# hccho2/Tacotron-Wavenet-Vocoder-Korean

Measured on AMD Instinct MI355X. Metric: WaveNet autoregressive audio samples/sec at 24 kHz, batch=8, higher is better.
Workload: dtype f32

## Files before the change

### tacotron-wavenet-vocoder-korean_amd/csrc/twv_wavenet_xcd.hip

```cpp
#include <hip/hip_runtime.h>
#include <stdint.h>
#include <string>
#include <type_traits>
#include "../../include/twv_amd.h"
#include "twv_layout.hpp"
#include "twv_math.hpp"
#include "twv_dev.hpp"
#include "twv_dpp.hpp"
#include "twv_categorical.hpp"
#include "twv_xcd.hpp"

using namespace twv;

#ifndef TWV_CHAIN_PAD
#define TWV_CHAIN_PAD 0
#endif
#ifndef TWV_WATCHDOG_LOG2
#define TWV_WATCHDOG_LOG2 21
#endif
#define TWV_STR2(x) #x
#define TWV_STR(x) TWV_STR2(x)
namespace {

typedef __attribute__((address_space(1))) unsigned long long gu64;
// ... 23 lines not shown
    return xb_load(rs, uword, lword);
}
__device__ __forceinline__ unsigned long long xbm_load(rsrc_t rs, int uword, int lword) { return xb_load_t<true>(rs, uword, lword); }
__device__ __forceinline__ u32x4s xbm_load2(rsrc_t rs, int uword, int lpair)
{
    asm volatile("" ::: "memory");
    return xb_load2(rs, uword, lpair);
}
__device__ __forceinline__ void xb_store(rsrc_t rs, int uword, int lword, unsigned tag, float v)
{
    __builtin_amdgcn_raw_buffer_store_b64(u32x2v{__float_as_uint(v), tag}, rs, lword * 8, uword * 8, kAuxStore);
    asm volatile("" ::: "memory");
}
__device__ __forceinline__ void xb_store2(rsrc_t rs, int uword, int lane, unsigned tag, float va, float vb)
{
    const u32x4s d = {__float_as_uint(va), tag, __float_as_uint(vb), tag};
    __builtin_amdgcn_raw_buffer_store_b128(d, rs, lane * 16, uword * 8, kAuxStore);
    asm volatile("s_nop 1" ::"v"(d) : "memory");
}
__device__ __forceinline__ unsigned g_tag(unsigned long long q) { return (unsigned)(q >> 32); }
__device__ __forceinline__ float g_val(unsigned long long q) { return __uint_as_float((unsigned)q); }

struct Poll {
    rsrc_t rs;
    int* status;
    int it;
    bool dead;
};
template <bool BAR = false>
__device__ __forceinline__ bool poll_tick(Poll& p, int code)
{
    if (p.dead) return false;
    if (((++p.it) & 63) == 0) {
        if (xb_load_t<BAR>(p.rs, (int)XcdExch::CTRL + 1, 0) != 0ull) { p.dead = true; return false; }
        if (p.it > (1 << TWV_WATCHDOG_LOG2)) {
            atomicMax(p.status, code);
            xb_store(p.rs, (int)XcdExch::CTRL + 1, 0, 1u, 0.0f);
            p.dead = true;
            return false;
        }
    }
    return true;
}
__device__ __forceinline__ void nap_until(unsigned long long target)
{
#pragma nounroll
    for (int i = 0; i < 4096 && __builtin_amdgcn_s_memtime() < target; ++i) __builtin_amdgcn_s_sleep(8);
}

__device__ __forceinline__ int lane_of_z(int k) { return ((k & 2) ? 16 : 0) + 2 * (k >> 2) + (k & 1); }
__device__ __forceinline__ int lane_of_x(int j) { return j < 16 ? j : 16 + j; }

struct ChainRegs { float wc[32]; float bd; };

#define XSTAMP(cond_, slot_) do { if ((INSTR & 1) && a.prof != nullptr && b == a.prof_stream && t < a.prof_steps && lane == 0 && (cond_)) a.prof[(long long)t * 64 + (slot_)] = wall_clock64(); } while (0)

#define WACC_DECL() unsigned long long wacc_[6] = {0, 0, 0, 0, 0, 0}, w0_ = 0, wt0_ = 0; if (INSTR & 4) wt0_ = __builtin_amdgcn_s_memtime()
#define WACC_T0() do { if (INSTR & 4) w0_ = __builtin_amdgcn_s_memtime(); } while (0)
#define WACC_T1(i_) do { if (INSTR & 4) wacc_[i_] += __builtin_amdgcn_s_memtime() - w0_; } while (0)
constexpr int kTraceStep = 2000;
#define WTRACE(cond_, slot_) do { if ((INSTR & 4) && a.prof != nullptr && t == kTraceStep && (cond_) && lane == 0) a.prof[2048 + (slot_)] = wall_clock64(); } while (0)
#define WACC_OUT(prof_, slot_, wave_) do { if ((INSTR & 4) && (prof_) != nullptr && (slot_) >= 0 && lane == 0) {                 \
        unsigned long long* o_ = (prof_) + (((slot_) * 8 + (wave_)) * 8);                                                        \
        o_[0] = __builtin_amdgcn_s_memtime() - wt0_;                                                                             \
        o_[1] = wacc_[0]; o_[2] = wacc_[1]; o_[3] = wacc_[2]; o_[4] = wacc_[3]; o_[5] = wacc_[4]; o_[6] = wacc_[5]; } } while (0)
#define XMARK(role_, stage_) do { if ((INSTR & 1) && lane == 0) xb_store(rs, (int)XcdExch::MARK + (role_) * 8 + (int)(threadIdx.x >> 6), 0, (unsigned)t + 1u, (float)(stage_)); } while (0)

enum { ROLE_CHAIN = 0, ROLE_SERVICE = 1, ROLE_SKIP0 = 2, ROLE_CONV0 = 10, ROLE_LC0 = 18 };
constexpr int kXcdStreamsPerXcd = kXcdStreams / 8;

struct XArgs {
    XcdLaunch p;
    int n_lc_wg, lc_lpw;
    int total_roles;
};

template <int NS> struct XStreams { rsrc_t rs[NS]; int b[NS]; };
__device__ __forceinline__ rsrc_t exch_rsrc(const XcdLaunch& a, int b)
{
    return __builtin_amdgcn_make_buffer_rsrc(a.exch + (long long)b * XcdExch::WORDS, 0, (int)(XcdExch::WORDS * 8), 0x00020000);
}
struct XLazyRs { const XcdLaunch* a; int xcc, ns; __device__ __forceinline__ rsrc_t operator[](int k) const { return exch_rsrc(*a, xcc + 8 * (k < ns ? k : 0)); } };
struct XLazyB { int xcc, ns; __device__ __forceinline__ int operator[](int k) const { return xcc + 8 * (k < ns ? k : 0); } };
template <int NS> struct XStreamsLazy { XLazyRs rs; XLazyB b; };
constexpr int kSkipLdsWords = 32 * 64;
constexpr int kConvLdsFloats = 16 * 64 + 64;

template <int INSTR, bool ALL, bool FORCED, bool SEG1, bool TWOSEG, int NC, bool ONEHOT = false, int HW = -1>
__device__ __forceinline__ void chain_role(const XArgs& xa, int b, rsrc_t rs)
{
    const XcdLaunch& a = xa.p;
    const Layout& L = a.lay;
    const int w = __builtin_amdgcn_readfirstlane(threadIdx.x >> 6), lane = threadIdx.x & 63;
    const int NL = L.NL, T = a.T;
    const bool use_bias = L.use_bias != 0, has_gc = L.G > 0, has_lc = L.L > 0;
    constexpr bool forced = FORCED;
    const int l0 = SEG1 ? kXcdSeg0Layers + 4 * w : (w < 6 ? 4 * w : 24 + 3 * (w - 6));
    const int lw0 = SEG1 ? 4 * w : l0;
    const int cap = SEG1 ? 4 : (w < 6 ? 4 : 3);
    int nl = NL - l0;
    nl = nl < 0 ? 0 : (nl > cap ? cap : nl);
    const int nlc = NC >= 0 ? NC : nl;
    const bool next_has = (l0 + nl < NL);
    const bool head = HW >= 0 ? (HW == 1) : (!SEG1 && (w == 7));
    const bool to_seg1 = TWOSEG && !SEG1 && w == 7 && next_has;
    constexpr bool two_seg = TWOSEG;
    if (nl == 0 && !head) return;
    const int oc = dpp_conv_out(lane), od = dpp_dense_out(lane);
    const ActCoef coef = act_coef(lane >= 32);
    float* stb = a.state + (long long)b * L.state_stride;
    Poll pl{rs, a.status, 0, false};
    constexpr int O_WD = 2048;

    ChainRegs W[4];
#pragma unroll
    for (int i = 0; i < 4; ++i) {
        if (i < nl) {
            const f32x4* src = reinterpret_cast<const f32x4*>(a.P + L.off_xl + (long long)(l0 + i) * kXcdXlFloats) + lane;
#pragma unroll
            for (int q = 0; q < 8; ++q) { const f32x4 v = src[q * 64]; W[i].wc[4 * q] = v.x; W[i].wc[4 * q + 1] = v.y; W[i].wc[4 * q + 2] = v.z; W[i].wc[4 * q + 3] = v.w; }
#pragma unroll
            for (int q = 0; q < 4; ++q) LDS4((O_WD >> 2) + ((lw0 + i) * 4 + q) * 64 + lane) = src[(8 + q) * 64];
            const f32x4 v = src[12 * 64];
            W[i].bd = dense_bias_init(lane, use_bias ? v.y : 0.0f);
        }
    }
    float ha = 0.0f, hb = 0.0f, first_in = 0.0f, b2v = 0.0f, s_lnl = 0.0f, s_tq = 0.0f, samp = 0.0f;
    float cp[4] = {0.0f, 0.0f, 0.0f, 0.0f};
    int q_prev = 0, q_valid = 0, samp_q = 0, first_q = 0;
    float w0row = 0.0f;
    double u_next = 0.0;
    const int chx = dpp_dense_out(lane);
    const bool sampler = head && !forced;
    const bool is15 = (lane & 15) == 15;
    auto causal_prepare = [&]() {
        const float t1 = __int_as_float(__builtin_amdgcn_update_dpp(0, __float_as_int(ha), 0x101, 0xf, 0xf, true));
        const float b0 = __int_as_float(__builtin_amdgcn_update_dpp(0, __float_as_int(hb), 0x150, 0xf, 0xf, true));
        ha = is15 ? b0 : t1;
        hb = __int_as_float(__builtin_amdgcn_update_dpp(0, __float_as_int(hb), 0x101, 0xf, 0xf, true));
        causal_partial_dpp(W[3].wc, ha, hb, cp);
    };
    auto noise = [&](int t) {
        const float* up = a.uniforms + ((long long)b * T + t) * (L.nr_mix + 1);
        const float u = lane <= L.nr_mix ? up[lane] : 0.5f;
        s_lnl = log_e(-log_e(u));
        const float uu = __shfl(u, L.nr_mix);
        s_tq = log_e(uu) - log_e(1.0f - uu);
    };
    if (head) {
        if constexpr (ONEHOT) {
            const int* meta = reinterpret_cast<const int*>(stb + L.st_meta);
            q_valid = __builtin_amdgcn_readfirstlane(meta[M_PREV_VALID]);
            q_prev = __builtin_amdgcn_readfirstlane(meta[M_QPREV]) & (L.Q - 1);
            w0row = a.P[L.off_causal + (long long)q_prev * 32 + chx];
            if (!forced) first_q = reinterpret_cast<const int*>(a.first_input)[b];
        } else {
            const f32x4* src = reinterpret_cast<const f32x4*>(a.P + L.off_xc) + lane;
#pragma unroll
            for (int q = 0; q < 8; ++q) { const f32x4 v = src[q * 64]; W[3].wc[4 * q] = v.x; W[3].wc[4 * q + 1] = v.y; W[3].wc[4 * q + 2] = v.z; W[3].wc[4 * q + 3] = v.w; }
            ha = stb[L.st_hist + (lane & 15)];
            hb = stb[L.st_hist + 16 + (lane & 15)];
            if (!forced) first_in = reinterpret_cast<const float*>(a.first_input)[b];
            if (sampler && use_bias && lane < L.O) b2v = a.P[L.off_b2 + lane];
            causal_prepare();
        }
    }
    __builtin_amdgcn_s_waitcnt(0);
    asm volatile(".p2align 6\n\t.rept " TWV_STR(TWV_CHAIN_PAD) "\n\ts_nop 0\n\t.endr" ::: "memory");

    float X = 0.0f;
    unsigned long long t_in = 0, in_period = 0, now_in = 0;
    for (int t = 0; t < T && !pl.dead; ++t) {
        asm volatile(".p2align 6");
        const unsigned tag = (unsigned)t + 1u;
        if (head) {
            if (forced && t > 0) {
                pl.it = 0;
                for (;;) {
                    const unsigned long long q = two_seg ? xb_load(rs, (int)XcdExch::DONE, lane) : LDSU64(8 * 64 + lane);
                    if (__all(g_tag(q) == (unsigned)t)) break;
                    if (!poll_tick(pl, 35)) break;
                    __builtin_amdgcn_s_sleep(2);
                }
                if (pl.dead) break;
            }
            XSTAMP(true, 0);
            if constexpr (ONEHOT) {
                const int q_raw = forced ? reinterpret_cast<const int*>(a.forced)[(long long)b * T + t] : (t == 0 ? first_q : samp_q);
                const int q_in = __builtin_amdgcn_readfirstlane(q_raw) & (L.Q - 1);
                const float w1row = a.P[L.off_causal + ((long long)L.Q + q_in) * 32 + chx];
                const float x0 = q_valid ? w0row + w1row : w1row;
                LDSU64(0 * 64 + lane) = ((unsigned long long)tag << 32) | (unsigned long long)__float_as_uint(x0);
                XSTAMP(true, 1);
                if (lane == 0) {
                    if (sampler && t > 0) reinterpret_cast<int*>(a.out)[(long long)b * T + t - 1] = samp_q;
                    xb_store(rs, (int)XcdExch::CTRL, 0, tag, 0.0f);
                }
                q_prev = q_in; q_valid = 1;
                w0row = a.P[L.off_causal + (long long)q_in * 32 + chx];
                if (sampler) u_next = reinterpret_cast<const double*>(a.uniforms)[(long long)b * T + t];
            } else {
            const float s_in = forced ? reinterpret_cast<const float*>(a.forced)[(long long)b * T + t] : (t == 0 ? first_in : samp);
            const float c3 = fma_(W[3].wc[31], s_in, cp[3]);
            const float x0 = (cp[0] + cp[1]) + (cp[2] + c3);
            LDSU64(0 * 64 + lane) = ((unsigned long long)tag << 32) | (unsigned long long)__float_as_uint(x0);
            XSTAMP(true, 1);
            if (lane == 0) {
                if (sampler && t > 0) a.out[(long long)b * T + t - 1] = samp;
                xb_store(rs, (int)XcdExch::CTRL, 0, tag, 0.0f);
            }
            hb = is15 ? s_in : hb;
            if (t + 1 < T) causal_prepare();
            if (sampler) noise(t);
            }
            __builtin_amdgcn_s_setprio(0);
        }
        XMARK(SEG1 ? 30 : ROLE_CHAIN, 1);
        float pre[4] = {0.0f, 0.0f, 0.0f, 0.0f};
        if (nlc > 0) {
            pl.it = 0;
            for (;;) {
                bool ok = true;
#pragma unroll
                for (int i = 0; i < 4; ++i) {
                    if (i < nlc) {
                        const unsigned long long qp = xb_load(rs, (int)XcdExch::PG + (l0 + i) * 64, oc);
                        ok = ok && g_tag(qp) == tag;
                        pre[i] = g_val(qp);
                    }
                }
                if (__all(ok)) break;
                if (!poll_tick(pl, 31)) break;
                __builtin_amdgcn_s_sleep(4);
            }
            XSTAMP(!SEG1, 26 + w);
            XMARK(SEG1 ? 30 : ROLE_CHAIN, 2);
            if (in_period) nap_until(t_in + in_period - (in_period >> 4));
            unsigned long long q;
            pl.it = 0;
            if (SEG1 && w == 0) {
                for (;;) {
                    q = xb_load(rs, (int)XcdExch::SEG, lane);
                    if (__all(g_tag(q) == tag)) break;
                    if (!poll_tick(pl, 36)) break;
                }
            } else {
                for (;;) {
                    q = LDSU64(w * 64 + lane);
                    if (__all(g_tag(q) == tag)) break;
                    if (!poll_tick(pl, 33)) break;
                }
            }
            __builtin_amdgcn_s_setprio(3);
            X = g_val(q);
            now_in = __builtin_amdgcn_s_memtime();
            XSTAMP(true, (SEG1 ? 40 : 2) + w);
            XMARK(SEG1 ? 30 : ROLE_CHAIN, 3);
        }
        constexpr bool DEFER = ALL && !FORCED && !SEG1 && NC > 0 && HW == 0;
        float zs[4] = {0.0f, 0.0f, 0.0f, 0.0f}, xs[4] = {0.0f, 0.0f, 0.0f, 0.0f};
        auto run_layers = [&](auto nc) {
            constexpr int N = decltype(nc)::value;
#pragma unroll
            for (int i = 0; i < N; ++i) {
                float wd[16];
#pragma unroll
                for (int q = 0; q < 4; ++q) {
                    const f32x4 v = LDS4((O_WD >> 2) + ((lw0 + i) * 4 + q) * 64 + lane);
                    wd[4 * q] = v.x; wd[4 * q + 1] = v.y; wd[4 * q + 2] = v.z; wd[4 * q + 3] = v.w;
                }
                const float z = layer_front_dpp(W[i].wc, coef, X, pre[i]);
                if (DEFER) { zs[i] = z; xs[i] = X; }
                else xb_store2(rs, (int)XcdExch::ZX + (l0 + i) * 128, lane, tag, z, X);
                layer_back_dpp(wd, W[i].bd, z, X);
                if ((INSTR & 2) && a.dbg != nullptr && t < a.dbg_steps) {
                    float* dp = a.dbg + ((long long)b * a.dbg_steps + t) * ((long long)NL * 64 + L.Opad) + (long long)(l0 + i) * 64;
                    if (lane < 32) dp[dpp_z_index(lane)] = z;
                    if ((lane & 16) == 0) dp[32 + od] = X;
                }
            }
        };
        if constexpr (NC > 0) run_layers(std::integral_constant<int, NC>{});
        else {
            if (nl == 4) run_layers(std::integral_constant<int, 4>{});
            else if (nl == 3) run_layers(std::integral_constant<int, 3>{});
            else if (nl == 2) run_layers(std::integral_constant<int, 2>{});
            else if (nl == 1) run_layers(std::integral_constant<int, 1>{});
        }
        if (to_seg1) xb_store(rs, (int)XcdExch::SEG, lane, tag, X);
        else if (nlc > 0) LDSU64((next_has ? w + 1 : 9) * 64 + lane) = ((unsigned long long)tag << 32) | (unsigned long long)__float_as_uint(X);
        XSTAMP(DEFER && nl > 0, (SEG1 ? 48 : 10) + w);
        if (DEFER) {
#pragma unroll
            for (int i = 0; i < (NC > 0 ? NC : 0); ++i) xb_store2(rs, (int)XcdExch::ZX + (l0 + i) * 128, lane, tag, zs[i], xs[i]);
        }
        if (forced && nl > 0 && !next_has) {
            if (SEG1) xb_store(rs, (int)XcdExch::DONE, lane, tag, 0.0f);
            else LDSU64(8 * 64 + lane) = (unsigned long long)tag << 32;
        }
        if (nlc > 0) {
            const unsigned long long d = now_in - t_in;
            in_period = (t_in != 0 && d < (1ull << 18)) ? d : 0;
            t_in = now_in;
        }
        if (!sampler) __builtin_amdgcn_s_setprio(0);
        XSTAMP(!DEFER && nl > 0, (SEG1 ? 48 : 10) + w);
        XMARK(SEG1 ? 30 : ROLE_CHAIN, 4);
        if constexpr (ONEHOT) {
          if (sampler) {
            __builtin_amdgcn_s_setprio(3);
            u32x4s d0, d1;
            pl.it = 0;
            for (;;) {
                d0 = xb_load2(rs, (int)XcdExch::QL, lane * 2);
                d1 = xb_load2(rs, (int)XcdExch::QL, lane * 2 + 1);
                if (__all(d0.y == tag && d0.w == tag && d1.y == tag && d1.w == tag)) break;
                if (!poll_tick(pl, 34)) break;
            }
            XSTAMP(true, 18);
            XMARK(SEG1 ? 30 : ROLE_CHAIN, 5);
            const float y[4] = {__uint_as_float(d0.x), __uint_as_float(d0.z), __uint_as_float(d1.x), __uint_as_float(d1.z)};
            if ((INSTR & 2) && a.dbg != nullptr && t < a.dbg_steps) {
#pragma unroll
                for (int k = 0; k < 4; ++k)
                    a.dbg[((long long)b * a.dbg_steps + t) * ((long long)NL * 64 + L.Opad) + (long long)NL * 64 + lane + 64 * k] = y[k];
            }
            bool bad_p = false;
            samp_q = categorical_sample<4>(y, L.Q, lane, a.temperature, u_next, nullptr,
                                           ((INSTR & 1) && a.prof != nullptr && b == a.prof_stream && t < a.prof_steps) ? a.prof + (long long)t * 64 + 38 : nullptr, &bad_p);
            if (bad_p && lane == 0) atomicMax(a.status, 31);
            XSTAMP(true, 19);
          }
        } else
        if (sampler) {
            __builtin_amdgcn_s_setprio(3);
            const int half = lane >> 5;
            unsigned long long q[8];
            pl.it = 0;
            for (;;) {
                bool good = true;
#pragma unroll
                for (int k = 0; k < 4; ++k) {
                    const u32x4s d = xb_load2(rs, (int)XcdExch::PT, (half * 4 + k) * 32 + (lane & 31));
                    q[2 * k] = ((unsigned long long)d.y << 32) | d.x;
                    q[2 * k + 1] = ((unsigned long long)d.w << 32) | d.z;
                    good = good && d.y == tag && d.w == tag;
                }
                if (__all(good)) break;
                if (!poll_tick(pl, 34)) break;
            }
            XSTAMP(true, 18);
            XMARK(SEG1 ? 30 : ROLE_CHAIN, 5);
            float y = g_val(q[0]);
#pragma unroll
            for (int k = 1; k < 8; ++k) y = y + g_val(q[k]);
#pragma unroll
            for (int k = 0; k < 8; ++k) {
                const auto sw = __builtin_amdgcn_permlane32_swap((unsigned)q[k], (unsigned)q[k], false, false);
                y = y + __uint_as_float(sw[1]);
            }
            if (use_bias && lane < L.O) y = y + b2v;
            if ((INSTR & 2) && a.dbg != nullptr && t < a.dbg_steps)
                a.dbg[((long long)b * a.dbg_steps + t) * ((long long)NL * 64 + L.Opad) + (long long)NL * 64 + lane] = y;
            const int nr = L.nr_mix;
            const float lsmin = (float)-32.23619130191664;
            const float e_all = exp_e(y > lsmin ? y : lsmin);
            const float ninf = __uint_as_float(0xff800000u);
            const float gmb = (lane < nr) ? y - s_lnl : ninf;
            float mx = gmb;
            mx = fmaxf(mx, __int_as_float(__builtin_amdgcn_update_dpp(__float_as_int(ninf), __float_as_int(mx), 0x111, 0xf, 0xf, false)));
            mx = fmaxf(mx, __int_as_float(__builtin_amdgcn_update_dpp(__float_as_int(ninf), __float_as_int(mx), 0x112, 0xf, 0xf, false)));
            mx = fmaxf(mx, __int_as_float(__builtin_amdgcn_update_dpp(__float_as_int(ninf), __float_as_int(mx), 0x114, 0xf, 0xf, false)));
            mx = fmaxf(mx, __int_as_float(__builtin_amdgcn_update_dpp(__float_as_int(ninf), __float_as_int(mx), 0x118, 0xf, 0xf, false)));
            const float best = __int_as_float(__builtin_amdgcn_readlane(__float_as_int(mx), 15));
            const unsigned long long hit = __ballot(lane < nr && gmb == best);
            const int k = hit ? (int)__ffsll((long long)hit) - 1 : 0;
            const float mean = __int_as_float(__builtin_amdgcn_readlane(__float_as_int(y), nr + k));
            const float e = __int_as_float(__builtin_amdgcn_readlane(__float_as_int(e_all), 2 * nr + k));
            const float prod = e * s_tq;
            float xs = mean + prod;
            xs = xs > -1.0f ? xs : -1.0f;
            xs = xs < 1.0f ? xs : 1.0f;
            samp = xs;
            XSTAMP(true, 19);
        }
    }

    if (head) {
        if constexpr (ONEHOT) {
            if (lane == 0) {
                if (sampler && !pl.dead && T > 0) reinterpret_cast<int*>(a.out)[(long long)b * T + T - 1] = samp_q;
                int* meta = reinterpret_cast<int*>(stb + L.st_meta);
                meta[M_TABS] = meta[M_TABS] + T;
                meta[M_PREV_VALID] = q_valid;
                meta[M_QPREV] = q_prev;
            }
        } else {
        if (sampler && !pl.dead && T > 0 && lane == 0) a.out[(long long)b * T + T - 1] = samp;
        if (lane < 16) stb[L.st_hist + lane] = ha;
        else if (lane < 32) stb[L.st_hist + lane] = hb;
        if (lane == 0) {
            int* meta = reinterpret_cast<int*>(stb + L.st_meta);
            meta[M_TABS] = meta[M_TABS] + T;
// ... 692 lines not shown
            lds[o_cur + lane] = rowa[k];
            lds[o_cur + 64 + lane] = rowb[k];
            if (mode != XLC_UPSAMPLED) {
#pragma unroll
                for (int i = 0; i < 4; ++i) {
                    if (i < n_up) {
                        const int o_nxt = (o_cur == o_row) ? o_row + 128 : o_row;
#pragma unroll
                        for (int hlf = 0; hlf < 2; ++hlf) {
                            const int m = hlf * 64 + lane;
                            const float x0 = lds[o_cur + m];
                            const float x1 = m > 0 ? lds[o_cur + m - 1] : 0.0f;
                            const float s0 = fma_(k0[i], x0, 0.0f);
                            const float s1 = fma_(k1[i], x1, 0.0f);
                            const float r = (s0 + s1) + (0.0f + 0.0f);
                            lds[o_nxt + m] = m < Lc ? r : 0.0f;
                        }
                        o_cur = o_nxt;
                    }
                }
            }
            float resx[kLt];
#pragma unroll
            for (int idx = 0; idx < kLt; ++idx) {
                resx[idx] = 0.0f;
                if (idx < nown * NLC) {
                    const int j = idx / NLC, c = idx - j * NLC;
                    const float xa_ = lds[o_cur + c * 32 + n16], xb_ = lds[o_cur + c * 32 + 16 + n16];
                    resx[idx] = dot32_dpp(lt[idx].w, xa_, xb_);
                    (void)j;
                }
            }
#pragma unroll
            for (int j = 0; j < kLt; ++j) {
                if (j < nown) {
                    float r = 0.0f;
#pragma unroll
                    for (int idx = 0; idx < kLt; ++idx) {
                        if (idx >= j * NLC && idx < (j + 1) * NLC) r = (idx == j * NLC) ? resx[idx] : r + resx[idx];
                    }
                    const int l = lfirst + j;
                    if (u + 1 < T) xb_store(rs, (int)XcdExch::LCR + (((u + 1) % kXcdLcRing) * kXcdLs + l) * 64, lane, (unsigned)u + 2u, r);
                    else {
                        if (T <= kXcdLcRing + 1) {
                            pl.rs = rs;
                            pl.it = 0;
                            for (;;) {
                                const unsigned long long ql = xb_load_t<BAR>(rs, (int)XcdExch::PG + l * 64, lane);
                                if (__all(g_tag(ql) >= 1u)) break;
                                if (!poll_tick<BAR>(pl, 73)) break;
                                __builtin_amdgcn_s_sleep(8);
                            }
                        }
                        (a.state + (long long)b * L.state_stride)[L.st_lcprev + l * 64 + lane] = r;
                    }
                }
            }
        }
        if (mode != XLC_UPSAMPLED) {
            int carry = 1;
            for (int i = n_up - 1; i >= 0; --i) {
                if (carry) { ph[i] += 1; carry = 0; if (ph[i] == L.up[i]) { ph[i] = 0; carry = 1; } }
            }
            frame += carry;
        }
    }
    if (pl.dead && lane == 0) {
#pragma unroll
        for (int k = 0; k < NS; ++k) xb_store(sx.rs[k], (int)XcdExch::CTRL + 1, 0, 1u, 0.0f);
    }
    WACC_OUT(a.prof, prof_slot, v);
}

__device__ __forceinline__ bool roles_resident(const XArgs& xa)
{
    const XcdLaunch& a = xa.p;
    __shared__ int s_go;
    if (threadIdx.x == 0) {
        int* arrived = a.roles + 8;
        int* decision = a.roles + 9;
        const int* hdr = reinterpret_cast<const int*>(a.cond);
        if (hdr[XH_MAGIC] != kXcdCondMagic || (unsigned)hdr[XH_MODE] > (unsigned)XLC_MEL) {
            atomicMax(a.status, 74);
            atomicCAS(decision, 0, 2);
        }
        if (atomicAdd(arrived, 1) + 1 == xa.total_roles) atomicCAS(decision, 0, 1);
        int f = 0;
#pragma nounroll
        for (int i = 0; i < (1 << 15); ++i) {
            f = atomicAdd(decision, 0);
            if (f != 0) break;
            __builtin_amdgcn_s_sleep(32);
        }
        if (f == 0) {
            const int old = atomicCAS(decision, 0, 2);
            f = old == 0 ? 2 : old;
            if (old == 0) atomicMax(a.status, 90);
        }
        s_go = (f == 1) ? 1 : 0;
    }
    __syncthreads();
    return s_go != 0;
}

template <int INSTR, bool BIGK, bool ONE, bool ONEHOT = false>
__global__ void __launch_bounds__(512) wn_xcd_generate_kernel(XArgs xa)
{
    const XcdLaunch& a = xa.p;
    unsigned xcc;
    asm volatile("s_getreg_b32 %0, hwreg(HW_REG_XCC_ID)" : "=s"(xcc));
    xcc &= 15u;
    int ticket = 0;
    if (threadIdx.x == 0) ticket = (xcc < (unsigned)a.B && xcc < 8u) ? atomicAdd(a.roles + xcc, 1) : 1 << 20;
    ticket = __shfl(ticket, 0);
    __shared__ int s_ticket;
    if (threadIdx.x == 0) s_ticket = ticket;
    for (int i = threadIdx.x; i < kXcdStreamsPerXcd * kSkipLdsWords * 2 + 64; i += blockDim.x) lds[i] = 0.0f;
    __syncthreads();
    ticket = s_ticket;
    const int ns = xcc < (unsigned)a.B && xcc < 8u ? (a.B - (int)xcc + 7) / 8 : 0;
    constexpr int nseg = BIGK ? 2 : 1;
    const int nchain = ns * nseg;
    if (ticket >= nchain + ns + 16 + xa.n_lc_wg) return;
    if (!roles_resident(xa)) return;
    const bool forced = a.forced != nullptr;
    auto exch_of = [&](int b) { return __builtin_amdgcn_make_buffer_rsrc(a.exch + (long long)b * XcdExch::WORDS, 0, (int)(XcdExch::WORDS * 8), 0x00020000); };
    if (ticket < nchain + ns) {
        const int k = ticket < nchain ? ticket / nseg : ticket - nchain;
        const int b = (int)xcc + 8 * k;
        const rsrc_t rs = exch_of(b);
        if (ticket < nchain) {
            if (ticket % nseg == 0) {
                const int wv = __builtin_amdgcn_readfirstlane(threadIdx.x >> 6);
                const int nlw = a.lay.NL - (wv < 6 ? 4 * wv : 24 + 3 * (wv - 6));
                if (forced) chain_role<INSTR, true, true, false, BIGK, -1, ONEHOT>(xa, b, rs);
                else if (nlw >= 4 && wv < 6) chain_role<INSTR, true, false, false, BIGK, 4, ONEHOT, 0>(xa, b, rs);
                else if (nlw >= 3 && wv == 6) chain_role<INSTR, true, false, false, BIGK, 3, ONEHOT, 0>(xa, b, rs);
                else if (nlw >= 3 && wv == 7) chain_role<INSTR, true, false, false, BIGK, 3, ONEHOT, 1>(xa, b, rs);
                else chain_role<INSTR, true, false, false, BIGK, -1, ONEHOT>(xa, b, rs);
            } else if constexpr (BIGK) {
                const int wv = __builtin_amdgcn_readfirstlane(threadIdx.x >> 6);
                if (forced) chain_role<INSTR, true, true, true, true, -1>(xa, b, rs);
                else if (a.lay.NL - kXcdSeg0Layers - 4 * wv >= 4) chain_role<INSTR, true, false, true, true, 4>(xa, b, rs);
                else chain_role<INSTR, true, false, true, true, -1>(xa, b, rs);
            }
        }
        else service_role<INSTR, BIGK>(xa, b, rs);
        return;
    }
    const int role = ticket - nchain - ns;
    auto shared_roles = [&](auto nsc) {
        constexpr int NS = decltype(nsc)::value;
        XStreams<NS> sx;
#pragma unroll
        for (int k = 0; k < NS; ++k) { sx.b[k] = (int)xcc + 8 * k; sx.rs[k] = exch_of(sx.b[k]); }
        constexpr int KF = TWV_XCD_KF;
        constexpr bool kUnfolded = KF == 0 || INSTR == 0;
        const bool fold = KF > 0 && (a.lay.NL > KF || !kUnfolded);
        if (role < 8) {
            if (!forced) {
                if (fold) skip_role<INSTR, NS, BIGK, KF>(xa, sx, role);
                else if constexpr (kUnfolded) skip_role<INSTR, NS, BIGK, 0>(xa, sx, role);
            }
        }
        else if (role < 16) {
            if (!forced) {
                if constexpr (ONEHOT) {
                    if (fold) conv1_onehot_role<INSTR, NS, KF>(xa, sx, role - 8);
                    else if constexpr (kUnfolded) conv1_onehot_role<INSTR, NS, 0>(xa, sx, role - 8);
                }
                else if (fold) conv1_role<INSTR, NS, false, XStreams<NS>, KF>(xa, sx, role - 8);
                else if constexpr (kUnfolded) conv1_role<INSTR, NS>(xa, sx, role - 8);
            }
        }
        else lc_role<INSTR, NS, BIGK>(xa, sx, role - 16);
    };
    if constexpr (BIGK) {
        if (ns == 1) shared_roles(std::integral_constant<int, 1>{});
        else shared_roles(std::integral_constant<int, 2>{});
    } else if constexpr (ONE) {
        shared_roles(std::integral_constant<int, 1>{});
    } else {
        if (ns == 1) shared_roles(std::integral_constant<int, 1>{});
        else if (ns == 2) shared_roles(std::integral_constant<int, 2>{});
        else if (ns == 3) shared_roles(std::integral_constant<int, 3>{});
        else shared_roles(std::integral_constant<int, 4>{});
    }
}

#define MMARK(rs_, slot_, stage_) do { if ((INSTR & 2) && lane == 0) xb_store(rs_, (int)XcdExch::MARK + (slot_), 0, (unsigned)t + 1u, (float)(stage_)); } while (0)
constexpr int kMS = 2;
constexpr int kManyChains = 6;
constexpr int kManyPerXcd = kMS * kManyChains;
constexpr int kM_BOX = 10;
constexpr int kM_OWD = 4096;
constexpr int kM_OGC = kM_OWD + kXcdSeg0Layers * 1024;
// ... 840 lines not shown
            dst[L.off_xl + i] = v;
        } else {
            const int e = (int)(i - per_layer * L.NL);
            const int q = e >> 8, lane = (e >> 2) & 63, c = e & 3;
            const int k = 4 * q + c;
            if (k < L.ifw) v = blob[L.c_causal + k * 32 + dpp_dense_out(lane)];
            dst[L.off_xc + e] = v;
        }
    }
}

}

namespace twv {

bool xcd_model_ok(const Layout& L)
{
    const bool head_ok = L.scalar ? (L.ifw == 32 && L.O <= 32 && L.NOJ == 1) : (L.Q == 256 && L.O == 256);
    return head_ok && L.S == 512 && L.NL >= 1 && L.NL <= kXcdMaxLayers && L.NLC <= 4;
}
static bool xcd_many_lc_fits(const Layout& L) { return (long long)kManyPerXcd * (L.n_up + 1) * L.NLC * 32 <= kManyLds / 8; }
int xcd_max_streams(const Layout& L) { return L.NL > kXcdSeg0Layers ? kXcdStreams / 2 : (L.scalar && xcd_many_lc_fits(L) ? kXcdManyStreams : kXcdStreams); }
static int lc_layers_per_wave(const Layout& L) { const int n = L.NLC > 0 ? (L.NL > kXcdSeg0Layers ? 6 : 4) / L.NLC : 1; return n < 1 ? 1 : (n > 4 ? 4 : n); }
int xcd_lc_workgroups(const Layout& L)
{
    if (L.L == 0) return 0;
    const int lpw = lc_layers_per_wave(L);
    const int waves = (L.NL + lpw - 1) / lpw;
    return (waves + 7) / 8;
}
int xcd_workgroups_per_stream(const Layout& L) { return ROLE_LC0 + xcd_lc_workgroups(L); }
size_t xcd_exchange_bytes(int batch) { return (size_t)batch * XcdExch::WORDS * 8 + 64; }
void xcd_pack(float* packed, const float* blob, const Layout& L, hipStream_t st)
{
    hipLaunchKernelGGL(wn_xcd_pack_kernel, dim3(512), dim3(256), 0, st, packed, blob, L);
}
bool xcd_uses_many(const Layout& L, int batch, int many_opt)
{
    return L.scalar && (batch > kXcdStreams || many_opt == 1 || (many_opt == 0 && batch >= kXcdManyFrom)) && L.NL <= kXcdSeg0Layers && xcd_many_lc_fits(L);
}
int xcd_launch(const XcdLaunch& p, hipStream_t st)
{
    XArgs xa;
    xa.p = p;
    xa.n_lc_wg = xcd_lc_workgroups(p.lay);
    xa.lc_lpw = lc_layers_per_wave(p.lay);
    const bool many = xcd_uses_many(p.lay, p.B, p.many);
    xa.total_roles = 0;
    for (int x = 0; x < 8 && x < p.B; ++x) {
        const int ns = (p.B - x + 7) / 8;
        if (many) xa.total_roles += 2 * ((ns + kMS - 1) / kMS) + 16 + xa.n_lc_wg;
        else xa.total_roles += ns * (p.lay.NL > kXcdSeg0Layers ? 2 : 1) + ns + 16 + xa.n_lc_wg;
    }
    const size_t shm = many ? (size_t)kManyLds * 4 : p.lay.NL > kXcdSeg0Layers ? (size_t)159 * 1024 : (size_t)(2048 + 32 * 1024) * 4;
    int dev = 0, cus = 256;
    hipDeviceProp_t prop;
    if (hipGetDevice(&dev) == hipSuccess && hipGetDeviceProperties(&prop, dev) == hipSuccess) cus = prop.multiProcessorCount;
    else (void)hipGetLastError();
    const int grid = 2 * cus;
    const int instr = (p.prof != nullptr ? 1 : 0) | (p.dbg != nullptr ? 2 : 0);
    auto go = [&](auto kern) {
        (void)hipFuncSetAttribute((const void*)kern, hipFuncAttributeMaxDynamicSharedMemorySize, (int)shm);
        (void)hipGetLastError();
        hipLaunchKernelGGL(kern, dim3(grid), dim3(512), shm, st, xa);
    };
    if (!many && instr != 0 && p.lay.NL <= TWV_XCD_KF)
        return twv_fail(TWV_E_UNSUPPORTED, "layer dumps / phase stamps of the XCD kernel need a model of at least two layers (set option \"xcd\" = 0 for the generic kernel)");
    if (many) {
        if (p.B > kXcdManyStreams) return twv_fail(TWV_E_UNSUPPORTED, "the many-streams XCD kernel takes at most 96 streams");
        if (instr == 3) return twv_fail(TWV_E_UNSUPPORTED, "layer dumps and wait accounting are separate builds of the many-streams kernel");
        if (instr == 1) go(wn_xcd_many_kernel<4>);
        else if (instr == 2) go(wn_xcd_many_kernel<2>);
        else go(wn_xcd_many_kernel<0>);
    }
    else if (!p.lay.scalar) {
        if (p.B > (p.lay.NL > kXcdSeg0Layers ? kXcdStreams / 2 : kXcdStreams)) return twv_fail(TWV_E_UNSUPPORTED, "the one-hot XCD kernel takes at most 32 streams (16 above 30 layers)");
        if (instr == 3 || (instr != 0 && p.lay.NL > kXcdSeg0Layers))
            return twv_fail(TWV_E_UNSUPPORTED, "the one-hot XCD kernel has layer dumps OR phase stamps, up to 30 layers (set option \"xcd\" = 0 for the generic kernel)");
        if (p.lay.NL > kXcdSeg0Layers) go(wn_xcd_generate_kernel<0, true, false, true>);
        else if (instr == 2) go(wn_xcd_generate_kernel<2, false, false, true>);
        else if (instr == 1) go(wn_xcd_generate_kernel<1, false, false, true>);
        else if (p.B <= 8) go(wn_xcd_generate_kernel<0, false, true, true>);
        else go(wn_xcd_generate_kernel<0, false, false, true>);
    }
    else if (p.lay.NL > kXcdSeg0Layers) {
        if (instr != 0) return twv_fail(TWV_E_UNSUPPORTED, "layer dumps / phase stamps exist for the 30-layer XCD kernel only (set option \"xcd\" = 0 for the generic kernel)");
        go(wn_xcd_generate_kernel<0, true, false>);
    }
    else if (instr == 3) go(wn_xcd_generate_kernel<3, false, false>);
    else if (instr == 2) go(wn_xcd_generate_kernel<2, false, false>);
    else if (instr == 1) go(wn_xcd_generate_kernel<1, false, false>);
    else if (p.B <= 8) go(wn_xcd_generate_kernel<0, false, true>);
    else go(wn_xcd_generate_kernel<0, false, false>);
    const hipError_t e = hipGetLastError();
    if (e != hipSuccess) return twv_fail(TWV_E_HIP, std::string("xcd launch: ") + hipGetErrorString(e));
    return TWV_OK;
}

}
```

### tacotron-wavenet-vocoder-korean_amd/csrc/twv_xcd.hpp

```cpp
#pragma once
#include <hip/hip_runtime.h>
#include <stddef.h>
#include <stdint.h>
#include "twv_layout.hpp"

namespace twv {

constexpr int kXcdSeg0Layers = 30;
constexpr int kXcdMaxLayers = 50;
constexpr int kXcdLs = 64;
constexpr int kXcdStreams = 32;
constexpr int kXcdManyFrom = 21;
constexpr int kXcdManyStreams = 96;
constexpr int kXcdLcRing = 16;
#ifndef TWV_MANY_LC_RING
#define TWV_MANY_LC_RING 8
#endif
constexpr int kXcdManyLcRing = TWV_MANY_LC_RING;
constexpr int kXcdXlFloats = 13 * 64 * 4;
constexpr int kXcdXcFloats = 8 * 64 * 4;

enum { XH_MAGIC = 0, XH_MODE = 1, XH_ROWS = 2, XH_WORDS = 64 };
constexpr int kXcdCondMagic = 0x58434431;
enum { XLC_NONE = 0, XLC_UPSAMPLED = 1, XLC_MEL = 2 };

struct XcdExch {
    static constexpr long long ZX = 0;
    static constexpr long long PG = ZX + kXcdLs * 128;
    static constexpr long long LG = PG + kXcdLs * 64;
    static constexpr long long H1 = LG + kXcdLs * 64;
    static constexpr long long PT = H1 + 512;
    static constexpr long long LCR = PT + 512;
    static constexpr long long CTRL = LCR + (long long)kXcdLcRing * kXcdLs * 64;
    static constexpr long long MARK = CTRL + 64;
    static constexpr long long SEG = MARK + 256;
    static constexpr long long DONE = SEG + 64;
    static constexpr long long SKT = DONE + 64;
    static constexpr long long H2 = SKT + 3 * 2 * 256;
    static constexpr long long QL = H2 + 512;
    static constexpr long long WORDS = QL + 256;
};

struct XcdLaunch {
    const float* P;
    float* state;
    const float* cond;
    const void* first_input;
    const void* forced;
    const float* uniforms;
    float temperature;
    float* out;
    int* status;
    float* dbg;
    int dbg_steps;
    unsigned long long* prof;
    int prof_steps;
    int prof_stream;
    int B, T;
    int many;
    unsigned long long* exch;
// ... 15 lines not shown
```

Measured before the change: 939,500.

## Repartition chain layers five per wave with a dedicated head wave

```diff
diff --git a/tacotron-wavenet-vocoder-korean_amd/csrc/twv_wavenet_xcd.hip b/tacotron-wavenet-vocoder-korean_amd/csrc/twv_wavenet_xcd.hip
--- a/tacotron-wavenet-vocoder-korean_amd/csrc/twv_wavenet_xcd.hip
+++ b/tacotron-wavenet-vocoder-korean_amd/csrc/twv_wavenet_xcd.hip
@@ -99,6 +99,56 @@
 __device__ __forceinline__ int lane_of_x(int j) { return j < 16 ? j : 16 + j; }
 
 struct ChainRegs { float wc[32]; float bd; };
+__device__ __forceinline__ void dot32_dpp_chain_lo(const float (&w)[16], float xa, float init, float (&c)[4])
+{
+    float c0 = init, c1, c2, c3;
+    asm volatile(
+        "s_nop 1\n" TWV_ALIGN8
+        "v_fmac_f32_dpp %0, %4, %5 row_newbcast:0 row_mask:0xf bank_mask:0xf\n"
+        "v_mul_f32_dpp %1, %4, %6 row_newbcast:1 row_mask:0xf bank_mask:0xf\n"
+        "v_mul_f32_dpp %2, %4, %7 row_newbcast:2 row_mask:0xf bank_mask:0xf\n"
+        "v_mul_f32_dpp %3, %4, %8 row_newbcast:3 row_mask:0xf bank_mask:0xf\n"
+        "v_fmac_f32_dpp %0, %4, %9 row_newbcast:4 row_mask:0xf bank_mask:0xf\n"
+        "v_fmac_f32_dpp %1, %4, %10 row_newbcast:5 row_mask:0xf bank_mask:0xf\n"
+        "v_fmac_f32_dpp %2, %4, %11 row_newbcast:6 row_mask:0xf bank_mask:0xf\n"
+        "v_fmac_f32_dpp %3, %4, %12 row_newbcast:7 row_mask:0xf bank_mask:0xf\n"
+        "v_fmac_f32_dpp %0, %4, %13 row_newbcast:8 row_mask:0xf bank_mask:0xf\n"
+        "v_fmac_f32_dpp %1, %4, %14 row_newbcast:9 row_mask:0xf bank_mask:0xf\n"
+        "v_fmac_f32_dpp %2, %4, %15 row_newbcast:10 row_mask:0xf bank_mask:0xf\n"
+        "v_fmac_f32_dpp %3, %4, %16 row_newbcast:11 row_mask:0xf bank_mask:0xf\n"
+        "v_fmac_f32_dpp %0, %4, %17 row_newbcast:12 row_mask:0xf bank_mask:0xf\n"
+        "v_fmac_f32_dpp %1, %4, %18 row_newbcast:13 row_mask:0xf bank_mask:0xf\n"
+        "v_fmac_f32_dpp %2, %4, %19 row_newbcast:14 row_mask:0xf bank_mask:0xf\n"
+        "v_fmac_f32_dpp %3, %4, %20 row_newbcast:15 row_mask:0xf bank_mask:0xf"
+        : "+v"(c0), "=&v"(c1), "=&v"(c2), "=&v"(c3)
+        : "v"(xa), "v"(w[0]), "v"(w[1]), "v"(w[2]), "v"(w[3]), "v"(w[4]), "v"(w[5]), "v"(w[6]), "v"(w[7]), "v"(w[8]), "v"(w[9]), "v"(w[10]), "v"(w[11]), "v"(w[12]), "v"(w[13]), "v"(w[14]), "v"(w[15]));
+    c[0] = c0; c[1] = c1; c[2] = c2; c[3] = c3;
+}
+__device__ __forceinline__ float dot32_dpp_chain_hi(const float (&w)[16], float xb, const float (&c)[4])
+{
+    float c0 = c[0], c1 = c[1], c2 = c[2], c3 = c[3];
+    asm volatile(
+        TWV_ALIGN8
+        "v_fmac_f32_dpp %0, %4, %5 row_newbcast:0 row_mask:0xf bank_mask:0xf\n"
+        "v_fmac_f32_dpp %1, %4, %6 row_newbcast:1 row_mask:0xf bank_mask:0xf\n"
+        "v_fmac_f32_dpp %2, %4, %7 row_newbcast:2 row_mask:0xf bank_mask:0xf\n"
+        "v_fmac_f32_dpp %3, %4, %8 row_newbcast:3 row_mask:0xf bank_mask:0xf\n"
+        "v_fmac_f32_dpp %0, %4, %9 row_newbcast:4 row_mask:0xf bank_mask:0xf\n"
+        "v_fmac_f32_dpp %1, %4, %10 row_newbcast:5 row_mask:0xf bank_mask:0xf\n"
+        "v_fmac_f32_dpp %2, %4, %11 row_newbcast:6 row_mask:0xf bank_mask:0xf\n"
+        "v_fmac_f32_dpp %3, %4, %12 row_newbcast:7 row_mask:0xf bank_mask:0xf\n"
+        "v_fmac_f32_dpp %0, %4, %13 row_newbcast:8 row_mask:0xf bank_mask:0xf\n"
+        "v_fmac_f32_dpp %1, %4, %14 row_newbcast:9 row_mask:0xf bank_mask:0xf\n"
+        "v_fmac_f32_dpp %2, %4, %15 row_newbcast:10 row_mask:0xf bank_mask:0xf\n"
+        "v_fmac_f32_dpp %3, %4, %16 row_newbcast:11 row_mask:0xf bank_mask:0xf\n"
+        "v_fmac_f32_dpp %0, %4, %17 row_newbcast:12 row_mask:0xf bank_mask:0xf\n"
+        "v_fmac_f32_dpp %1, %4, %18 row_newbcast:13 row_mask:0xf bank_mask:0xf\n"
+        "v_fmac_f32_dpp %2, %4, %19 row_newbcast:14 row_mask:0xf bank_mask:0xf\n"
+        "v_fmac_f32_dpp %3, %4, %20 row_newbcast:15 row_mask:0xf bank_mask:0xf"
+        : "+v"(c0), "+v"(c1), "+v"(c2), "+v"(c3)
+        : "v"(xb), "v"(w[0]), "v"(w[1]), "v"(w[2]), "v"(w[3]), "v"(w[4]), "v"(w[5]), "v"(w[6]), "v"(w[7]), "v"(w[8]), "v"(w[9]), "v"(w[10]), "v"(w[11]), "v"(w[12]), "v"(w[13]), "v"(w[14]), "v"(w[15]));
+    return (c0 + c1) + (c2 + c3);
+}
 
 #define XSTAMP(cond_, slot_) do { if ((INSTR & 1) && a.prof != nullptr && b == a.prof_stream && t < a.prof_steps && lane == 0 && (cond_)) a.prof[(long long)t * 64 + (slot_)] = wall_clock64(); } while (0)
 
@@ -133,7 +183,8 @@
 constexpr int kSkipLdsWords = 32 * 64;
 constexpr int kConvLdsFloats = 16 * 64 + 64;
 
-template <int INSTR, bool ALL, bool FORCED, bool SEG1, bool TWOSEG, int NC, bool ONEHOT = false, int HW = -1>
+constexpr int kChainLpw = 5;
+template <int INSTR, bool ALL, bool FORCED, bool SEG1, bool TWOSEG, int NC, bool ONEHOT = false, bool HEAD = false, bool CONT = false>
 __device__ __forceinline__ void chain_role(const XArgs& xa, int b, rsrc_t rs)
 {
     const XcdLaunch& a = xa.p;
@@ -142,15 +193,16 @@
     const int NL = L.NL, T = a.T;
     const bool use_bias = L.use_bias != 0, has_gc = L.G > 0, has_lc = L.L > 0;
     constexpr bool forced = FORCED;
-    const int l0 = SEG1 ? kXcdSeg0Layers + 4 * w : (w < 6 ? 4 * w : 24 + 3 * (w - 6));
-    const int lw0 = SEG1 ? 4 * w : l0;
-    const int cap = SEG1 ? 4 : (w < 6 ? 4 : 3);
+    constexpr int kLayerWaves = kXcdSeg0Layers / kChainLpw;
+    const int l0 = (SEG1 ? kXcdSeg0Layers : 0) + kChainLpw * w;
+    const int lw0 = kChainLpw * w;
+    const int cap = (HEAD || w >= kLayerWaves) ? 0 : kChainLpw;
     int nl = NL - l0;
     nl = nl < 0 ? 0 : (nl > cap ? cap : nl);
     const int nlc = NC >= 0 ? NC : nl;
     const bool next_has = (l0 + nl < NL);
-    const bool head = HW >= 0 ? (HW == 1) : (!SEG1 && (w == 7));
-    const bool to_seg1 = TWOSEG && !SEG1 && w == 7 && next_has;
+    constexpr bool head = HEAD;
+    const bool to_seg1 = TWOSEG && !SEG1 && w == kLayerWaves - 1 && next_has;
     constexpr bool two_seg = TWOSEG;
     if (nl == 0 && !head) return;
     const int oc = dpp_conv_out(lane), od = dpp_dense_out(lane);
@@ -158,20 +210,27 @@
     float* stb = a.state + (long long)b * L.state_stride;
     Poll pl{rs, a.status, 0, false};
     constexpr int O_WD = 2048;
-
-    ChainRegs W[4];
-#pragma unroll
-    for (int i = 0; i < 4; ++i) {
-        if (i < nl) {
+    constexpr int O_WH = kXcdChainHalfTiles;
+
+    float wlo[kChainLpw - 1][16], whi[kChainLpw][16], bdi[kChainLpw];
+#pragma unroll
+    for (int i = 0; i < kChainLpw; ++i) {
+        if (!HEAD && i < nl) {
             const f32x4* src = reinterpret_cast<const f32x4*>(a.P + L.off_xl + (long long)(l0 + i) * kXcdXlFloats) + lane;
 #pragma unroll
-            for (int q = 0; q < 8; ++q) { const f32x4 v = src[q * 64]; W[i].wc[4 * q] = v.x; W[i].wc[4 * q + 1] = v.y; W[i].wc[4 * q + 2] = v.z; W[i].wc[4 * q + 3] = v.w; }
+            for (int q = 0; q < 4; ++q) {
+                const f32x4 lo = src[q * 64], hi = src[(4 + q) * 64];
+                if (i == 0) LDS4((O_WH >> 2) + (w * 4 + q) * 64 + lane) = lo;
+                else { wlo[i > 0 ? i - 1 : 0][4 * q] = lo.x; wlo[i > 0 ? i - 1 : 0][4 * q + 1] = lo.y; wlo[i > 0 ? i - 1 : 0][4 * q + 2] = lo.z; wlo[i > 0 ? i - 1 : 0][4 * q + 3] = lo.w; }
+                whi[i][4 * q] = hi.x; whi[i][4 * q + 1] = hi.y; whi[i][4 * q + 2] = hi.z; whi[i][4 * q + 3] = hi.w;
+            }
 #pragma unroll
             for (int q = 0; q < 4; ++q) LDS4((O_WD >> 2) + ((lw0 + i) * 4 + q) * 64 + lane) = src[(8 + q) * 64];
             const f32x4 v = src[12 * 64];
-            W[i].bd = dense_bias_init(lane, use_bias ? v.y : 0.0f);
-        }
-    }
+            bdi[i] = dense_bias_init(lane, use_bias ? v.y : 0.0f);
+        }
+    }
+    float wcz[32];
     float ha = 0.0f, hb = 0.0f, first_in = 0.0f, b2v = 0.0f, s_lnl = 0.0f, s_tq = 0.0f, samp = 0.0f;
     float cp[4] = {0.0f, 0.0f, 0.0f, 0.0f};
     int q_prev = 0, q_valid = 0, samp_q = 0, first_q = 0;
@@ -185,7 +244,7 @@
         const float b0 = __int_as_float(__builtin_amdgcn_update_dpp(0, __float_as_int(hb), 0x150, 0xf, 0xf, true));
         ha = is15 ? b0 : t1;
         hb = __int_as_float(__builtin_amdgcn_update_dpp(0, __float_as_int(hb), 0x101, 0xf, 0xf, true));
-        causal_partial_dpp(W[3].wc, ha, hb, cp);
+        causal_partial_dpp(wcz, ha, hb, cp);
     };
     auto noise = [&](int t) {
         const float* up = a.uniforms + ((long long)b * T + t) * (L.nr_mix + 1);
@@ -204,7 +263,7 @@
         } else {
             const f32x4* src = reinterpret_cast<const f32x4*>(a.P + L.off_xc) + lane;
 #pragma unroll
-            for (int q = 0; q < 8; ++q) { const f32x4 v = src[q * 64]; W[3].wc[4 * q] = v.x; W[3].wc[4 * q + 1] = v.y; W[3].wc[4 * q + 2] = v.z; W[3].wc[4 * q + 3] = v.w; }
+            for (int q = 0; q < 8; ++q) { const f32x4 v = src[q * 64]; wcz[4 * q] = v.x; wcz[4 * q + 1] = v.y; wcz[4 * q + 2] = v.z; wcz[4 * q + 3] = v.w; }
             ha = stb[L.st_hist + (lane & 15)];
             hb = stb[L.st_hist + 16 + (lane & 15)];
             if (!forced) first_in = reinterpret_cast<const float*>(a.first_input)[b];
@@ -217,6 +276,7 @@
 
     float X = 0.0f;
     unsigned long long t_in = 0, in_period = 0, now_in = 0;
+    unsigned long long t_tab = 0, tab_period = 0, now_tab = 0;
     for (int t = 0; t < T && !pl.dead; ++t) {
         asm volatile(".p2align 6");
         const unsigned tag = (unsigned)t + 1u;
@@ -248,7 +308,7 @@
                 if (sampler) u_next = reinterpret_cast<const double*>(a.uniforms)[(long long)b * T + t];
             } else {
             const float s_in = forced ? reinterpret_cast<const float*>(a.forced)[(long long)b * T + t] : (t == 0 ? first_in : samp);
-            const float c3 = fma_(W[3].wc[31], s_in, cp[3]);
+            const float c3 = fma_(wcz[31], s_in, cp[3]);
             const float x0 = (cp[0] + cp[1]) + (cp[2] + c3);
             LDSU64(0 * 64 + lane) = ((unsigned long long)tag << 32) | (unsigned long long)__float_as_uint(x0);
             XSTAMP(true, 1);
@@ -260,16 +320,22 @@
             if (t + 1 < T) causal_prepare();
             if (sampler) noise(t);
             }
+            if (sampler) {
+                const unsigned long long d = now_tab - t_tab;
+                tab_period = (t_tab != 0 && d < (1ull << 18)) ? d : 0;
+                t_tab = now_tab;
+            }
             __builtin_amdgcn_s_setprio(0);
         }
         XMARK(SEG1 ? 30 : ROLE_CHAIN, 1);
-        float pre[4] = {0.0f, 0.0f, 0.0f, 0.0f};
+        float pre[kChainLpw] = {0.0f, 0.0f, 0.0f, 0.0f, 0.0f};
+        float w0lo[16];
         if (nlc > 0) {
             pl.it = 0;
             for (;;) {
                 bool ok = true;
 #pragma unroll
-                for (int i = 0; i < 4; ++i) {
+                for (int i = 0; i < kChainLpw; ++i) {
                     if (i < nlc) {
                         const unsigned long long qp = xb_load(rs, (int)XcdExch::PG + (l0 + i) * 64, oc);
                         ok = ok && g_tag(qp) == tag;
@@ -283,6 +349,12 @@
             XSTAMP(!SEG1, 26 + w);
             XMARK(SEG1 ? 30 : ROLE_CHAIN, 2);
             if (in_period) nap_until(t_in + in_period - (in_period >> 4));
+            asm volatile("" ::: "memory");
+#pragma unroll
+            for (int k = 0; k < 4; ++k) {
+                const f32x4 v = LDS4((O_WH >> 2) + (w * 4 + k) * 64 + lane);
+                w0lo[4 * k] = v.x; w0lo[4 * k + 1] = v.y; w0lo[4 * k + 2] = v.z; w0lo[4 * k + 3] = v.w;
+            }
             unsigned long long q;
             pl.it = 0;
             if (SEG1 && w == 0) {
@@ -304,22 +376,28 @@
             XSTAMP(true, (SEG1 ? 40 : 2) + w);
             XMARK(SEG1 ? 30 : ROLE_CHAIN, 3);
         }
-        constexpr bool DEFER = ALL && !FORCED && !SEG1 && NC > 0 && HW == 0;
-        float zs[4] = {0.0f, 0.0f, 0.0f, 0.0f}, xs[4] = {0.0f, 0.0f, 0.0f, 0.0f};
+        constexpr bool DEFER = ALL && !FORCED && !SEG1 && NC > 0 && CONT;
+        float zs[kChainLpw] = {0.0f, 0.0f, 0.0f, 0.0f, 0.0f}, xs[kChainLpw] = {0.0f, 0.0f, 0.0f, 0.0f, 0.0f};
         auto run_layers = [&](auto nc) {
             constexpr int N = decltype(nc)::value;
 #pragma unroll
             for (int i = 0; i < N; ++i) {
+                const auto xab = __builtin_amdgcn_permlane32_swap(__float_as_uint(X), __float_as_uint(X), false, false);
+                float cc[4];
+                dot32_dpp_chain_lo(i == 0 ? w0lo : wlo[i > 0 ? i - 1 : 0], __uint_as_float(xab[0]), pre[i], cc);
+                asm volatile("" ::: "memory");
                 float wd[16];
 #pragma unroll
                 for (int q = 0; q < 4; ++q) {
                     const f32x4 v = LDS4((O_WD >> 2) + ((lw0 + i) * 4 + q) * 64 + lane);
                     wd[4 * q] = v.x; wd[4 * q + 1] = v.y; wd[4 * q + 2] = v.z; wd[4 * q + 3] = v.w;
                 }
-                const float z = layer_front_dpp(W[i].wc, coef, X, pre[i]);
+                const float act = act_eval_pk_med3(coef, dot32_dpp_chain_hi(whi[i], __uint_as_float(xab[1]), cc));
+                const auto sw = __builtin_amdgcn_permlane32_swap(__float_as_uint(act), __float_as_uint(act), false, false);
+                const float z = __uint_as_float(sw[0]) * __uint_as_float(sw[1]);
                 if (DEFER) { zs[i] = z; xs[i] = X; }
                 else xb_store2(rs, (int)XcdExch::ZX + (l0 + i) * 128, lane, tag, z, X);
-                layer_back_dpp(wd, W[i].bd, z, X);
+                layer_back_dpp(wd, bdi[i], z, X);
                 if ((INSTR & 2) && a.dbg != nullptr && t < a.dbg_steps) {
                     float* dp = a.dbg + ((long long)b * a.dbg_steps + t) * ((long long)NL * 64 + L.Opad) + (long long)(l0 + i) * 64;
                     if (lane < 32) dp[dpp_z_index(lane)] = z;
@@ -329,7 +407,8 @@
         };
         if constexpr (NC > 0) run_layers(std::integral_constant<int, NC>{});
         else {
-            if (nl == 4) run_layers(std::integral_constant<int, 4>{});
+            if (nl == 5) run_layers(std::integral_constant<int, 5>{});
+            else if (nl == 4) run_layers(std::integral_constant<int, 4>{});
             else if (nl == 3) run_layers(std::integral_constant<int, 3>{});
             else if (nl == 2) run_layers(std::integral_constant<int, 2>{});
             else if (nl == 1) run_layers(std::integral_constant<int, 1>{});
@@ -355,6 +434,7 @@
         XMARK(SEG1 ? 30 : ROLE_CHAIN, 4);
         if constexpr (ONEHOT) {
           if (sampler) {
+            if (tab_period) nap_until(t_tab + tab_period - (tab_period >> 3));
             __builtin_amdgcn_s_setprio(3);
             u32x4s d0, d1;
             pl.it = 0;
@@ -364,6 +444,7 @@
                 if (__all(d0.y == tag && d0.w == tag && d1.y == tag && d1.w == tag)) break;
                 if (!poll_tick(pl, 34)) break;
             }
+            now_tab = __builtin_amdgcn_s_memtime();
             XSTAMP(true, 18);
             XMARK(SEG1 ? 30 : ROLE_CHAIN, 5);
             const float y[4] = {__uint_as_float(d0.x), __uint_as_float(d0.z), __uint_as_float(d1.x), __uint_as_float(d1.z)};
@@ -380,6 +461,7 @@
           }
         } else
         if (sampler) {
+            if (tab_period) nap_until(t_tab + tab_period - (tab_period >> 3));
             __builtin_amdgcn_s_setprio(3);
             const int half = lane >> 5;
             unsigned long long q[8];
@@ -396,6 +478,7 @@
                 if (__all(good)) break;
                 if (!poll_tick(pl, 34)) break;
             }
+            now_tab = __builtin_amdgcn_s_memtime();
             XSTAMP(true, 18);
             XMARK(SEG1 ? 30 : ROLE_CHAIN, 5);
             float y = g_val(q[0]);
@@ -1194,7 +1277,9 @@
                                 __builtin_amdgcn_s_sleep(8);
                             }
                         }
-                        (a.state + (long long)b * L.state_stride)[L.st_lcprev + l * 64 + lane] = r;
+                        int off = L.st_lcprev + l * 64 + lane;
+                        if constexpr (BIG) asm volatile("" : "+v"(off));
+                        (a.state + (long long)b * L.state_stride)[off] = r;
                     }
                 }
             }
@@ -1274,16 +1359,20 @@
         if (ticket < nchain) {
             if (ticket % nseg == 0) {
                 const int wv = __builtin_amdgcn_readfirstlane(threadIdx.x >> 6);
-                const int nlw = a.lay.NL - (wv < 6 ? 4 * wv : 24 + 3 * (wv - 6));
-                if (forced) chain_role<INSTR, true, true, false, BIGK, -1, ONEHOT>(xa, b, rs);
-                else if (nlw >= 4 && wv < 6) chain_role<INSTR, true, false, false, BIGK, 4, ONEHOT, 0>(xa, b, rs);
-                else if (nlw >= 3 && wv == 6) chain_role<INSTR, true, false, false, BIGK, 3, ONEHOT, 0>(xa, b, rs);
-                else if (nlw >= 3 && wv == 7) chain_role<INSTR, true, false, false, BIGK, 3, ONEHOT, 1>(xa, b, rs);
+                const int nlw = a.lay.NL - kChainLpw * wv;
+                if (wv == 7) {
+                    if (forced) chain_role<INSTR, true, true, false, BIGK, 0, ONEHOT, true>(xa, b, rs);
+                    else chain_role<INSTR, true, false, false, BIGK, 0, ONEHOT, true>(xa, b, rs);
+                }
+                else if (wv >= kXcdSeg0Layers / kChainLpw || nlw <= 0) {}
+                else if (forced) chain_role<INSTR, true, true, false, BIGK, -1, ONEHOT>(xa, b, rs);
+                else if (nlw > kChainLpw) chain_role<INSTR, true, false, false, BIGK, kChainLpw, ONEHOT, false, true>(xa, b, rs);
+                else if (nlw == kChainLpw) chain_role<INSTR, true, false, false, BIGK, kChainLpw, ONEHOT, false, false>(xa, b, rs);
                 else chain_role<INSTR, true, false, false, BIGK, -1, ONEHOT>(xa, b, rs);
             } else if constexpr (BIGK) {
                 const int wv = __builtin_amdgcn_readfirstlane(threadIdx.x >> 6);
                 if (forced) chain_role<INSTR, true, true, true, true, -1>(xa, b, rs);
-                else if (a.lay.NL - kXcdSeg0Layers - 4 * wv >= 4) chain_role<INSTR, true, false, true, true, 4>(xa, b, rs);
+                else if (a.lay.NL - kXcdSeg0Layers - kChainLpw * wv >= kChainLpw) chain_role<INSTR, true, false, true, true, kChainLpw>(xa, b, rs);
                 else chain_role<INSTR, true, false, true, true, -1>(xa, b, rs);
             }
         }
@@ -2230,7 +2319,7 @@
         if (many) xa.total_roles += 2 * ((ns + kMS - 1) / kMS) + 16 + xa.n_lc_wg;
         else xa.total_roles += ns * (p.lay.NL > kXcdSeg0Layers ? 2 : 1) + ns + 16 + xa.n_lc_wg;
     }
-    const size_t shm = many ? (size_t)kManyLds * 4 : p.lay.NL > kXcdSeg0Layers ? (size_t)159 * 1024 : (size_t)(2048 + 32 * 1024) * 4;
+    const size_t shm = many ? (size_t)kManyLds * 4 : p.lay.NL > kXcdSeg0Layers ? (size_t)159 * 1024 : (size_t)kXcdChainLdsFloats * 4;
     int dev = 0, cus = 256;
     hipDeviceProp_t prop;
     if (hipGetDevice(&dev) == hipSuccess && hipGetDeviceProperties(&prop, dev) == hipSuccess) cus = prop.multiProcessorCount;
diff --git a/tacotron-wavenet-vocoder-korean_amd/csrc/twv_xcd.hpp b/tacotron-wavenet-vocoder-korean_amd/csrc/twv_xcd.hpp
--- a/tacotron-wavenet-vocoder-korean_amd/csrc/twv_xcd.hpp
+++ b/tacotron-wavenet-vocoder-korean_amd/csrc/twv_xcd.hpp
@@ -6,6 +6,8 @@
 
 namespace twv {
 
+constexpr int kXcdChainHalfTiles = 2048 + 30 * 1024;
+constexpr int kXcdChainLdsFloats = kXcdChainHalfTiles + 6 * 1024;
 constexpr int kXcdSeg0Layers = 30;
 constexpr int kXcdMaxLayers = 50;
 constexpr int kXcdLs = 64;
```

Result: faster. 972,900, median of 6 (+3.6%).
